# antgroup/ant-ray

Measured on NVIDIA H100. Metric: resnet50_ddp_train_images_per_sec, higher is better.
Workload: dtype bf16

## Files before the change

### ant-ray_b200/csrc/inst_norm.cu

```cuda
#include <algorithm>
#include <initializer_list>
#include <type_traits>

#include "norm_act.cuh"
#include "norm_infer.cuh"
#include "norm_kernels.cuh"
#include "norm_launch.h"
#include "norm_res.cuh"

namespace b200c {
namespace bn {

static int ceil_div(int a, int b) { return (a + b - 1) / b; }

static int last_pow2(unsigned n) {
  n |= (n >> 1);
  n |= (n >> 2);
  n |= (n >> 4);
  n |= (n >> 8);
  n |= (n >> 16);
  return std::max<int>(1, n - (n >> 1));
}

static void reduce_config(int reduction, int stride, dim3* block, dim3* grid) {
  int block_x = std::min(last_pow2(stride), kTileW);
  int block_y = std::min(last_pow2(ceil_div(reduction, kElemsPerThread)), kMaxBlock / block_x);
  if (block_x * block_y != kMaxBlock) block_x = std::min(last_pow2(stride), kMaxBlock / block_y);
  int grid_y = std::min(ceil_div(reduction, block_y * kElemsPerThread), kMaxHBlock);
  *block = dim3(block_x, block_y, 1);
  *grid = dim3(ceil_div(stride, block_x), grid_y < 8 ? 1 : grid_y, 1);
}

static_assert(kEwVec % kStatsVec == 0, "vec_ok covers the statistics kernel's vector width");
static bool vec_ok(int stride, const void* const* ptrs, int n) {
  if (stride % kEwVec) return false;
  for (int i = 0; i < n; i++)
    if (reinterpret_cast<uintptr_t>(ptrs[i]) % 16) return false;
  return true;
}

static void ew_config(int reduction, int stride, int vec, dim3* block, dim3* grid) {
  const int groups = stride / vec;
  const int bx = std::min(groups, kEwThreads);
  const int by = kEwThreads / bx;
  const int gx = ceil_div(groups, bx);
  const int gy = std::max(1, std::min(ceil_div(reduction, by), 4096 / gx));
  *block = dim3(bx, by, 1);
  *grid = dim3(gx, gy, 1);
}

constexpr int kSemaphores = kMaxChannels / kTileW;
constexpr size_t kSemaphoreBytes = (size_t)kSemaphores * 4;

// ... 18 lines not shown
template <int... Cs, typename F>
static auto with_const(int key, F&& f) {
  std::common_type_t<decltype(f(std::integral_constant<int, Cs>{}))...> kernel = nullptr;
  ((key == Cs ? void(kernel = f(std::integral_constant<int, Cs>{})) : void()), ...);
  return kernel;
}

using StatsKernel = void (*)(const bf16*, StatsOut, volatile float*, int*, int, int);
using SyncStatsKernel = void (*)(const bf16*, float*, float, volatile float*, int*, int, int);
using StatsDualKernel = void (*)(const bf16*, const bf16*, StatsOut, StatsOut, volatile float*, volatile float*, int*, int, int);
using TransformKernel = void (*)(const bf16*, const bf16*, bf16*, uint8_t*, const float*, const float*, const float*, const float*,
                                 const float*, const float*, const float*, const float*, int, int);
using PoolFwdKernel = void (*)(const bf16*, bf16*, uint8_t*, const float*, const float*, const float*, const float*, PoolDims, int, int);
using BwdReduceKernel = void (*)(const bf16*, const bf16*, const bf16*, const bf16*, const uint8_t*, bf16*, const float*, const float*,
                                 float*, float*, float*, float*, volatile float*, int*, PoolDims, const bf16*, const float*, const float*,
                                 float*, float*, float*, int, int);
using BwdElemtKernel = void (*)(const bf16*, const bf16*, const bf16*, const uint8_t*, const bf16*, bf16*, const float*, const float*,
                                const float*, const float*, const float*, const float*, float, const bf16*, bf16*, const float*,
                                const float*, const float*, const float*, int, int);

static StatsKernel stats_kernel(int vec) {
  return with_const<1, kStatsVec>(vec, [](auto v) -> StatsKernel { return k_bn_stats<decltype(v)::value>; });
}
static StatsDualKernel stats_dual_kernel(int vec) {
  return with_const<1, kStatsVec>(vec, [](auto v) -> StatsDualKernel { return k_bn_stats_dual<decltype(v)::value>; });
}
static SyncStatsKernel sync_stats_kernel(int vec) {
  return with_const<1, kStatsVec>(vec, [](auto v) -> SyncStatsKernel { return k_bn_sync_stats<decltype(v)::value>; });
}
static TransformKernel transform_kernel(int vec, int tail) {
  return with_const<1, kEwVec>(vec, [&](auto v) {
// ... 130 lines not shown
      load(res_infer_kernel<float>(vec, b));
      load(res_infer_kernel<bf16>(vec, b));
    }
  }
  return e;
}

constexpr cudaError_t kNoKernel = cudaErrorInvalidDeviceFunction;

static cudaError_t launch_stats(const FwdArgs& a, float* sync_row, cudaStream_t st) {
  Scratch s = carve(a.scratch, a.c);
  dim3 block, grid;
  reduce_config(a.m, a.c, &block, &grid);
  const int vec = vec_ok(a.c, &a.x, 1) ? kStatsVec : 1;
  block.x /= vec;
  const bf16* x = static_cast<const bf16*>(a.x);
  if (sync_row) {
    const SyncStatsKernel k = sync_stats_kernel(vec);
    if (!k) return kNoKernel;
    k<<<grid, block, 0, st>>>(x, sync_row, a.eps, s.staging, s.semaphores, a.m, a.c);
  } else {
    const StatsKernel k = stats_kernel(vec);
    if (!k) return kNoKernel;
    StatsOut o{a.save_mean, a.save_invstd, a.running_mean, a.running_var, a.num_batches_tracked, a.momentum,
               (float)((double)a.m / (double)(a.m - 1)), a.eps};
    k<<<grid, block, 0, st>>>(x, o, s.staging, s.semaphores, a.m, a.c);
  }
  return cudaGetLastError();
}

static cudaError_t launch_transform(const FwdArgs& a, cudaStream_t st) {
  const void* ptrs[3] = {a.x, a.y, a.identity ? a.identity : a.x};
  const int vec = vec_ok(a.c, ptrs, 3) ? kEwVec : 1;
  dim3 block, grid;
  ew_config(a.m, a.c, vec, &block, &grid);
  const TransformKernel k = transform_kernel(vec, !a.relu ? kTailNone : a.identity ? kTailAddRelu : kTailRelu);
  if (!k) return kNoKernel;
  k<<<grid, block, 0, st>>>(static_cast<const bf16*>(a.x), static_cast<const bf16*>(a.identity), static_cast<bf16*>(a.y),
                            static_cast<uint8_t*>(a.mask), a.save_mean, a.save_invstd, a.weight, a.bias, nullptr, nullptr, nullptr,
                            nullptr, a.m, a.c);
  return cudaGetLastError();
// ... 18 lines not shown
cudaError_t forward(const FwdArgs& a, cudaStream_t st) {
  const cudaError_t e = launch_stats(a, nullptr, st);
  if (e != cudaSuccess) return e;
  return a.pool_h ? launch_pool_fwd(a, st) : launch_transform(a, st);
}

static GradSrc grad_src(const BwdArgs& a, bool reduced) {
  if (!a.relu) return kGradDy;
  if (reduced && a.dy_masked) return kGradMasked;
  if (a.pool_h) return kGradPool;
  return a.mask ? kGradBits : kGradY;
}

static cudaError_t launch_bwd_reduce(const BwdArgs& a, cudaStream_t st) {
  Scratch s = carve(a.scratch, a.c);
  dim3 block, grid;
  reduce_config(a.m, a.c, &block, &grid);
  const GradSrc src = grad_src(a, false);
  const BwdReduceKernel k = bwd_reduce_kernel(src, false);
  if (!k) return kNoKernel;
  const void* mask = src == kGradPool ? a.argmax : a.mask;
  k<<<grid, block, 0, st>>>(static_cast<const bf16*>(a.x), static_cast<const bf16*>(a.dy), static_cast<const bf16*>(a.dy2),
                            static_cast<const bf16*>(a.y), static_cast<const uint8_t*>(mask), static_cast<bf16*>(a.dy_masked),
                            a.save_mean, a.save_invstd, s.sums, s.sums + a.c, a.grad_weight, a.grad_bias, s.staging, s.semaphores,
                            pool_dims(a.pool_h, a.pool_w), nullptr, nullptr, nullptr, nullptr, nullptr, nullptr, a.m, a.c);
  return cudaGetLastError();
}

static cudaError_t launch_bwd_elemt(const BwdArgs& a, cudaStream_t st) {
  Scratch s = carve(a.scratch, a.c);
  const GradSrc src = grad_src(a, true);
  const void* g = src == kGradMasked ? a.dy_masked : a.dy;
  const void* ptrs[5] = {a.x, a.dx, g, a.dy2 && src != kGradMasked ? a.dy2 : a.dy, a.y};
  const int vec = vec_ok(a.c, ptrs, src == kGradY ? 5 : 4) ? kEwVec : 1;
  dim3 block, grid;
  ew_config(a.m, a.c, vec, &block, &grid);
  const BwdElemtKernel k = bwd_elemt_kernel(vec, src, a.norm_fct != nullptr, false);
  if (!k) return kNoKernel;
  k<<<grid, block, 0, st>>>(static_cast<const bf16*>(g), static_cast<const bf16*>(a.dy2), static_cast<const bf16*>(a.y),
                            static_cast<const uint8_t*>(a.mask), static_cast<const bf16*>(a.x), static_cast<bf16*>(a.dx), a.save_mean,
// ... 8 lines not shown
}

static size_t dual_extra_offset(int c) { return (scratch_bytes(c) + 15) / 16 * 16; }
size_t dual_scratch_bytes(int c) { return dual_extra_offset(c) + (size_t)3 * c * kMaxHBlock * 4 + (size_t)c * 4; }
static float* dual_staging(void* scratch, int c) { return reinterpret_cast<float*>(static_cast<char*>(scratch) + dual_extra_offset(c)); }
static float* dual_sum_xmu2(void* scratch, int c) { return dual_staging(scratch, c) + (size_t)3 * c * kMaxHBlock; }

cudaError_t forward_dual(const FwdArgs& a, const FwdArgs& b, cudaStream_t st) {
  Scratch s = carve(a.scratch, a.c);
  dim3 block, grid;
  reduce_config(a.m, a.c, &block, &grid);
  const void* xs[2] = {a.x, b.x};
  const int svec = vec_ok(a.c, xs, 2) ? kStatsVec : 1;
  block.x /= svec;
  grid.z = 2;
  const StatsDualKernel ks = stats_dual_kernel(svec);
  if (!ks) return kNoKernel;
  StatsOut oa{a.save_mean, a.save_invstd, a.running_mean, a.running_var, a.num_batches_tracked, a.momentum,
              (float)((double)a.m / (double)(a.m - 1)), a.eps};
  StatsOut ob{b.save_mean, b.save_invstd, b.running_mean, b.running_var, b.num_batches_tracked, b.momentum,
              (float)((double)b.m / (double)(b.m - 1)), b.eps};
  ks<<<grid, block, 0, st>>>(static_cast<const bf16*>(a.x), static_cast<const bf16*>(b.x), oa, ob, s.staging,
                             dual_staging(a.scratch, a.c), s.semaphores, a.m, a.c);
  cudaError_t e = cudaGetLastError();
  if (e != cudaSuccess) return e;
  const void* ptrs[3] = {a.x, a.y, b.x};
  const int vec = vec_ok(a.c, ptrs, 3) ? kEwVec : 1;
  ew_config(a.m, a.c, vec, &block, &grid);
  const TransformKernel kt = transform_kernel(vec, kTailBnAddRelu);
  if (!kt) return kNoKernel;
  kt<<<grid, block, 0, st>>>(static_cast<const bf16*>(a.x), static_cast<const bf16*>(b.x), static_cast<bf16*>(a.y),
                             static_cast<uint8_t*>(a.mask), a.save_mean, a.save_invstd, a.weight, a.bias, b.save_mean, b.save_invstd,
                             b.weight, b.bias, a.m, a.c);
  return cudaGetLastError();
}

cudaError_t backward_dual(const BwdArgs& a, const BwdArgs& b, cudaStream_t st) {
  Scratch s = carve(a.scratch, a.c);
  float* sum2 = dual_sum_xmu2(a.scratch, a.c);
  const GradSrc src = a.mask ? kGradBits : kGradY;
  dim3 block, grid;
  reduce_config(a.m, a.c, &block, &grid);
  const BwdReduceKernel kr = bwd_reduce_kernel(src, true);
  if (!kr) return kNoKernel;
  kr<<<grid, block, 0, st>>>(static_cast<const bf16*>(a.x), static_cast<const bf16*>(a.dy), static_cast<const bf16*>(a.dy2),
                             static_cast<const bf16*>(a.y), static_cast<const uint8_t*>(a.mask), nullptr, a.save_mean, a.save_invstd,
                             s.sums, s.sums + a.c, a.grad_weight, a.grad_bias, s.staging, s.semaphores, pool_dims(0, 0),
                             static_cast<const bf16*>(b.x), b.save_mean, b.save_invstd, sum2, b.grad_weight, b.grad_bias, a.m, a.c);
  cudaError_t e = cudaGetLastError();
  if (e != cudaSuccess) return e;
  const void* ptrs[7] = {a.x, a.dx, a.dy, a.dy2 ? a.dy2 : a.dy, b.x, b.dx, a.y};
  const int vec = vec_ok(a.c, ptrs, src == kGradY ? 7 : 6) ? kEwVec : 1;
  ew_config(a.m, a.c, vec, &block, &grid);
  const BwdElemtKernel ke = bwd_elemt_kernel(vec, src, false, true);
  if (!ke) return kNoKernel;
  ke<<<grid, block, 0, st>>>(static_cast<const bf16*>(a.dy), static_cast<const bf16*>(a.dy2), static_cast<const bf16*>(a.y),
                             static_cast<const uint8_t*>(a.mask), static_cast<const bf16*>(a.x), static_cast<bf16*>(a.dx), a.save_mean,
                             a.save_invstd, a.weight, s.sums, s.sums + a.c, nullptr, (float)(1.0 / a.m), static_cast<const bf16*>(b.x),
                             static_cast<bf16*>(b.dx), b.save_mean, b.save_invstd, b.weight, sum2, a.m, a.c);
  return cudaGetLastError();
}

template <typename P>
static cudaError_t launch_infer(const InferArgs& a, cudaStream_t st) {
  auto p = [](const void* q) { return static_cast<const P*>(q); };
  const bf16* x = static_cast<const bf16*>(a.x);
  bf16* y = static_cast<bf16*>(a.y);
// ... 179 lines not shown
```

### ant-ray_b200/csrc/norm_kernels.cuh

```cuda
#pragma once
#include <cuda_bf16.h>
#include <cuda_runtime.h>
#include <stdint.h>

namespace b200c {
namespace bn {

constexpr int kMaxBlock = 512;
constexpr int kParallelLoads = 4;
constexpr int kElemsPerThread = 16;
constexpr int kTileW = 32;
constexpr int kMaxHBlock = 128;
constexpr int kStatsVec = 4;
constexpr int kEwThreads = 256;
constexpr int kEwVec = 8;

typedef __nv_bfloat16 bf16;

template <int V>
struct alignas(2 * V) BVec {
  bf16 v[V];
};


template <bool FUSE_NEW>
__device__ __forceinline__ void welford_merge_element(int& count, float& mean, float& m2n, const int& count_new,
                                                      const float& mean_new, const float& m2n_new) {
  float factor = float(1.0) / ::max(1, (count + count_new));
  float delta0 = mean - mean_new;
  const float c = count, c_new = count_new;
  mean = __fmul_rn(FUSE_NEW ? __fmaf_rn(mean_new, c_new, __fmul_rn(mean, c)) : __fmaf_rn(mean, c, __fmul_rn(mean_new, c_new)),
                   factor);
  m2n = __fadd_rn(m2n, __fmaf_rn(__fmul_rn(__fmul_rn(__fmul_rn(delta0, delta0), c_new), c), factor, m2n_new));
  count += count_new;
}

template <int V>
// ... 13 lines not shown
    }
    __syncthreads();
    if (threadIdx.y < offset && threadIdx.y + offset < blockDim.y) {
      auto address = address_base + offset * block_x;
#pragma unroll
      for (int k = 0; k < V; k++) {
        auto count_new = shmem_count[address + k];
        auto mean_new = shmem_mean[address + k];
        auto m2n_new = shmem_m2n[address + k];
        welford_merge_element<false>(count[k], mean[k], m2n[k], count_new, mean_new, m2n_new);
      }
    }
  }
}

__device__ __forceinline__ void merge_block_vertical_backward(float& sum_dy, float& sum_dy_xmu, float* shmem_sum_dy,
                                                              float* shmem_sum_dy_xmu) {
  auto address_base = threadIdx.x + threadIdx.y * blockDim.x;
#pragma unroll
  for (int offset = blockDim.y / 2; offset > 0; offset >>= 1) {
    if (threadIdx.y < offset * 2) {
      shmem_sum_dy[address_base] = sum_dy;
      shmem_sum_dy_xmu[address_base] = sum_dy_xmu;
    }
    __syncthreads();
    if (threadIdx.y < offset && threadIdx.y + offset < blockDim.y) {
      auto address = address_base + offset * blockDim.x;
      sum_dy += shmem_sum_dy[address];
      sum_dy_xmu += shmem_sum_dy_xmu[address];
    }
  }
}

struct StatsOut {
  float* save_mean;
  float* save_invstd;
  float* running_mean;
  float* running_var;
  long long* num_batches_tracked;
  float momentum, bessel, eps;
};

__device__ __forceinline__ void finish_stats(const StatsOut& o, int c, float mean_th, float m2_th, int count_th) {
  const float mean = mean_th;
  const float var = m2_th / count_th;
  const float momentum = o.momentum;
// ... 15 lines not shown
  for (int i = 0; i < PARALLEL_LOADS; i++) {
#pragma unroll
    for (int k = 0; k < V; k++) {
      x_mean[i][k] = 0.f;
      m_2_n[i][k] = 0.f;
    }
    count[i] = 0;
  }

  int inner_loop_stride = blockDim.y * gridDim.y;
  int m_offset = blockIdx.y * blockDim.y + threadIdx.y;
  int c_offset = (blockIdx.x * blockDim.x + threadIdx.x) * V;
  int loop_count = 1 + (reduction_size - 1) / (inner_loop_stride * PARALLEL_LOADS);
  const bool c_valid = c_offset < stride;

  for (int i = 0; i < loop_count; i++) {
    BVec<V> xv[PARALLEL_LOADS];
#pragma unroll
    for (int j = 0; j < PARALLEL_LOADS; j++) {
      const int m = m_offset + j * inner_loop_stride;
      if (c_valid && m < reduction_size) xv[j] = *reinterpret_cast<const BVec<V>*>(input + ((size_t)m * stride + c_offset));
    }
#pragma unroll
    for (int j = 0; j < PARALLEL_LOADS; j++) {
      float x_math[V];
      float x_count_inv;
      float is_valid;
      if (c_valid && m_offset < reduction_size) {
#pragma unroll
        for (int k = 0; k < V; k++) x_math[k] = __bfloat162float(xv[j].v[k]);
        count[j]++;
        x_count_inv = float(1) / count[j];
        is_valid = float(1);
      } else {
#pragma unroll
        for (int k = 0; k < V; k++) x_math[k] = float(0);
        x_count_inv = float(0);
        is_valid = float(0);
      }
      m_offset += inner_loop_stride;
#pragma unroll
      for (int k = 0; k < V; k++) {
        float delta0 = x_math[k] - x_mean[j][k];
        x_mean[j][k] = __fmaf_rn(delta0, x_count_inv, x_mean[j][k]);
        float delta1 = x_math[k] - x_mean[j][k];
        m_2_n[j][k] = __fmaf_rn(__fmul_rn(delta0, delta1), is_valid, m_2_n[j][k]);
      }
    }
  }
  float mean_th[V], m2_th[V];
  int count_th[V];
#pragma unroll
  for (int k = 0; k < V; k++) {
    count_th[k] = count[0];
    mean_th[k] = x_mean[0][k];
    m2_th[k] = m_2_n[0][k];
#pragma unroll
    for (int j = 1; j < PARALLEL_LOADS; j++) welford_merge_element<true>(count_th[k], mean_th[k], m2_th[k], count[j], x_mean[j][k], m_2_n[j][k]);
  }

  __shared__ float shmem_mean[kMaxBlock];
  __shared__ float shmem_m2n[kMaxBlock];
// ... 265 lines not shown
  if (a[0] == at) sum += __bfloat162float(v[0]);
  if (pw1 != pw0 && a[1] == at - 2) sum += __bfloat162float(v[1]);
  if (ph1 != ph0 && a[2] == at - 6) sum += __bfloat162float(v[2]);
  if (ph1 != ph0 && pw1 != pw0 && a[3] == at - 8) sum += __bfloat162float(v[3]);
  return __float2bfloat16(sum);
}

__device__ __forceinline__ bf16 relu_grad(bf16 dy, bf16 y) { return __bfloat162float(y) <= 0.f ? __float2bfloat16(0.f) : dy; }
__device__ __forceinline__ bf16 relu_grad_bit(bf16 dy, unsigned bit) { return bit ? dy : __float2bfloat16(0.f); }
__device__ __forceinline__ bf16 add_grads(bf16 a, bf16 b) { return __float2bfloat16(__bfloat162float(a) + __bfloat162float(b)); }

enum GradSrc { kGradMasked, kGradY, kGradBits, kGradDy, kGradPool };
constexpr int kGradSrcs = 5;

template <GradSrc G, bool DUAL>
__global__ void k_bn_bwd_reduce(const bf16* __restrict__ input, const bf16* __restrict__ grad_output,
                                const bf16* __restrict__ grad_output2, const bf16* __restrict__ output,
                                const uint8_t* __restrict__ mask, bf16* __restrict__ masked, const float* __restrict__ mean,
                                const float* __restrict__ inv_std, float* __restrict__ sum_dy_o, float* __restrict__ sum_dy_xmu_o,
                                float* __restrict__ grad_weight, float* __restrict__ grad_bias, volatile float* staging_data,
                                int* semaphores, const PoolDims pool, const bf16* __restrict__ input2,
                                const float* __restrict__ mean2, const float* __restrict__ inv_std2, float* __restrict__ sum_dy_xmu2_o,
                                float* __restrict__ grad_weight2, float* __restrict__ grad_bias2, const int reduction_size,
                                const int stride) {
  static_assert(G != kGradMasked, "the reduce kernel computes g");
  constexpr bool BITS = G == kGradBits;
  constexpr bool POOL = G == kGradPool;
  constexpr int PARALLEL_LOADS = kParallelLoads;
  float sum_dy[PARALLEL_LOADS];
  float sum_dy_xmu[PARALLEL_LOADS];
  float sum_dy_xmu2[PARALLEL_LOADS];
#pragma unroll
  for (int i = 0; i < PARALLEL_LOADS; i++) {
    sum_dy[i] = float(0);
    sum_dy_xmu[i] = float(0);
    sum_dy_xmu2[i] = float(0);
  }
  int inner_loop_stride = blockDim.y * gridDim.y;
  int m_offset = blockIdx.y * blockDim.y + threadIdx.y;
  int c_offset = blockIdx.x * blockDim.x + threadIdx.x;
  if (c_offset >= stride || m_offset >= reduction_size) return;

  int loop_count = 1 + (reduction_size - 1) / (inner_loop_stride * PARALLEL_LOADS);
  int address_base = m_offset * stride + c_offset;
  int address_increment = inner_loop_stride * stride;
  auto r_mean = mean[c_offset];
  auto factor = inv_std[c_offset];
  const float r_mean2 = DUAL ? mean2[c_offset] : 0.f;

  for (int i = 0; i < loop_count; i++) {
    bf16 dy_v[PARALLEL_LOADS], dy2_v[PARALLEL_LOADS], y_v[PARALLEL_LOADS], x_v[PARALLEL_LOADS], x2_v[PARALLEL_LOADS];
    uint8_t mask_v[PARALLEL_LOADS];
#pragma unroll
    for (int j = 0; j < PARALLEL_LOADS; j++) {
      if (m_offset + j * inner_loop_stride < reduction_size) {
        const int a = address_base + j * address_increment;
        if (POOL) dy_v[j] = pool_grad(grad_output, mask, pool, m_offset + j * inner_loop_stride, c_offset, stride);
        else dy_v[j] = grad_output[a];
        if (grad_output2) dy2_v[j] = grad_output2[a];
        if (BITS) mask_v[j] = mask[a >> 3];
        else if (G == kGradY) y_v[j] = output[a];
        x_v[j] = input[a];
        if (DUAL) x2_v[j] = input2[a];
      }
    }
    float x_input[PARALLEL_LOADS];
    float x_input2[PARALLEL_LOADS];
    float x_grad_output[PARALLEL_LOADS];
#pragma unroll
    for (int j = 0; j < PARALLEL_LOADS; j++) {
      if (c_offset < stride && m_offset < reduction_size) {
        const bf16 dy = !POOL && grad_output2 ? add_grads(dy_v[j], dy2_v[j]) : dy_v[j];
        const bf16 g = BITS ? relu_grad_bit(dy, (mask_v[j] >> (address_base & 7)) & 1u) : G == kGradY ? relu_grad(dy, y_v[j]) : dy;
        if (masked) masked[address_base] = g;
        x_input[j] = __bfloat162float(x_v[j]);
        x_input2[j] = DUAL ? __bfloat162float(x2_v[j]) : 0.f;
        x_grad_output[j] = __bfloat162float(g);
      } else {
        x_input[j] = float(0);
        x_input2[j] = float(0);
        x_grad_output[j] = float(0);
      }
      m_offset += inner_loop_stride;
      address_base += address_increment;
    }
#pragma unroll
    for (int j = 0; j < PARALLEL_LOADS; j++) {
      sum_dy[j] += x_grad_output[j];
      sum_dy_xmu[j] = __fmaf_rn(x_grad_output[j], x_input[j] - r_mean, sum_dy_xmu[j]);
      if (DUAL) sum_dy_xmu2[j] = __fmaf_rn(x_grad_output[j], x_input2[j] - r_mean2, sum_dy_xmu2[j]);
    }
  }
#pragma unroll
  for (int j = 1; j < PARALLEL_LOADS; j++) {
    sum_dy[0] += sum_dy[j];
    sum_dy_xmu[0] += sum_dy_xmu[j];
    if (DUAL) sum_dy_xmu2[0] += sum_dy_xmu2[j];
  }
  auto sum_dy_th = sum_dy[0];
  auto sum_dy_xmu_th = sum_dy_xmu[0];
  float sum_dy_xmu2_th = sum_dy_xmu2[0];

  __shared__ float shmem_sum_dy[kMaxBlock];
  __shared__ float shmem_sum_dy_xmu[kMaxBlock];
  auto merge = [&]() {
    merge_block_vertical_backward(sum_dy_th, sum_dy_xmu_th, shmem_sum_dy, shmem_sum_dy_xmu);
    if (DUAL) {
      __syncthreads();
      float unused = 0.f;
      merge_block_vertical_backward(sum_dy_xmu2_th, unused, shmem_sum_dy, shmem_sum_dy_xmu);
    }
  };
  merge();

  auto write_sums = [&]() {
    grad_bias[c_offset] = sum_dy_th;
    grad_weight[c_offset] = sum_dy_xmu_th * factor;
    sum_dy_o[c_offset] = sum_dy_th;
    sum_dy_xmu_o[c_offset] = sum_dy_xmu_th;
    if (DUAL) {
      grad_bias2[c_offset] = sum_dy_th;
      grad_weight2[c_offset] = sum_dy_xmu2_th * inv_std2[c_offset];
      sum_dy_xmu2_o[c_offset] = sum_dy_xmu2_th;
    }
  };
  if (gridDim.y > 1) {
    volatile float* staging_sum_dy = staging_data;
    volatile float* staging_sum_dy_xmu = &staging_data[stride * gridDim.y];
    volatile float* staging_sum_dy_xmu2 = &staging_data[2 * stride * gridDim.y];
    address_base = c_offset + blockIdx.y * stride;
    if (threadIdx.y == 0 && c_offset < stride) {
      staging_sum_dy[address_base] = sum_dy_th;
      staging_sum_dy_xmu[address_base] = sum_dy_xmu_th;
      if (DUAL) staging_sum_dy_xmu2[address_base] = sum_dy_xmu2_th;
    }
    __threadfence();
    __syncthreads();
    __shared__ bool is_last_block_done;
    if (threadIdx.x == 0 && threadIdx.y == 0) {
      int old = atomicAdd(&semaphores[blockIdx.x], 1);
      is_last_block_done = (old == (gridDim.y - 1));
      if (is_last_block_done) semaphores[blockIdx.x] = 0;
    }
    __syncthreads();
    if (is_last_block_done) {
      sum_dy_th = float(0.0);
      sum_dy_xmu_th = float(0.0);
      sum_dy_xmu2_th = float(0.0);
      for (int y = threadIdx.y; y < gridDim.y; y += blockDim.y) {
        address_base = c_offset + y * stride;
        sum_dy_th += (c_offset < stride ? staging_sum_dy[address_base] : float(0.0));
        sum_dy_xmu_th += (c_offset < stride ? staging_sum_dy_xmu[address_base] : float(0.0));
        if (DUAL) sum_dy_xmu2_th += (c_offset < stride ? staging_sum_dy_xmu2[address_base] : float(0.0));
      }
      merge();
      if (threadIdx.y == 0 && c_offset < stride) write_sums();
    }
  } else {
    if (blockIdx.y == 0 && threadIdx.y == 0 && c_offset < stride) write_sums();
  }
}

template <int V, GradSrc G, bool FCT_PTR, bool DUAL>
__global__ void __launch_bounds__(kEwThreads) k_bn_bwd_elemt(const bf16* __restrict__ grad_output, const bf16* __restrict__ grad_output2,
                                                             const bf16* __restrict__ output, const uint8_t* __restrict__ mask,
                                                             const bf16* __restrict__ input, bf16* __restrict__ grad_input,
                                                             const float* __restrict__ mean, const float* __restrict__ inv_std,
                                                             const float* __restrict__ weight, const float* __restrict__ sum_dy,
                                                             const float* __restrict__ sum_dy_xmu,
                                                             const float* __restrict__ norm_fct_ptr, const float norm_fct_value,
                                                             const bf16* __restrict__ input2, bf16* __restrict__ grad_input2,
                                                             const float* __restrict__ mean2, const float* __restrict__ inv_std2,
                                                             const float* __restrict__ weight2, const float* __restrict__ sum_dy_xmu2,
                                                             const int reduction_size, const int stride) {
  static_assert(!DUAL || (G == kGradY || G == kGradBits), "a dual tail derives g from dy and the ReLU");
// ... 48 lines not shown
```

Measured before the change: 5472.

## Pipeline BN stats and backward-reduce loads through cp.async shared-memory rings

The batch-norm statistics kernel and the backward reduce kernel now stage their global loads through a multi-stage shared-memory ring filled with cp.async, so loads for later iterations overlap with the Welford and gradient accumulation of the current one. The backward reduce kernel also gains a 4-wide channel vectorized path, selected at launch through a new vec argument, with dynamic shared memory sized by operand count. This aims to hide memory latency in these bandwidth-bound reductions. In exchange, each block uses more shared memory, which may lower occupancy, and the code adds more template paths.

Result: faster. 5648, median of 6 (+3.2%).

```diff
diff --git a/ant-ray_b200/csrc/inst_norm.cu b/ant-ray_b200/csrc/inst_norm.cu
--- a/ant-ray_b200/csrc/inst_norm.cu
+++ b/ant-ray_b200/csrc/inst_norm.cu
@@ -37,6 +37,38 @@
   for (int i = 0; i < n; i++)
     if (reinterpret_cast<uintptr_t>(ptrs[i]) % 16) return false;
   return true;
+}
+
+constexpr size_t kBlockSmem = 48 * 1024;
+constexpr size_t kStatsStaticSmem = 3 * kMaxBlock * 4 + 16;
+constexpr size_t kBwdStaticSmem = 2 * kMaxBlock * 4 + 16;
+
+static size_t stats_ring_bytes(dim3 block) {
+  return (size_t)kStatsStages * kParallelLoads * block.x * block.y * sizeof(BVec<kStatsVec>);
+}
+static_assert(kStatsStaticSmem + (size_t)kStatsStages * kParallelLoads * (kMaxBlock / kStatsVec) * sizeof(BVec<kStatsVec>) <= kBlockSmem,
+              "the statistics ring fits every block");
+
+static_assert(kBwdStaticSmem + (size_t)kBwdStagesWide * 5 * kParallelLoads * (kMaxBlock / kBwdVec) * sizeof(BVec<kBwdVec>) <= kBlockSmem &&
+                  kBwdStaticSmem + (size_t)kBwdStages * 2 * kParallelLoads * (kMaxBlock / kBwdVec) * sizeof(BVec<kBwdVec>) <= kBlockSmem,
+              "the backward ring fits every block: 2 stages of up to 5 operands, 3 of 2");
+struct BwdReduceLaunch {
+  dim3 block, grid;
+  int vec;
+  size_t smem;
+};
+static BwdReduceLaunch bwd_reduce_launch(int m, int c, GradSrc src, bool dy2, bool dual, const void* const* ptrs, int n) {
+  BwdReduceLaunch l;
+  reduce_config(m, c, &l.block, &l.grid);
+  l.vec = 1;
+  l.smem = 0;
+  if (src == kGradPool || !vec_ok(c, ptrs, n)) return l;
+  const int ops = bwd_ring_operands(src == kGradY, dy2, dual);
+  const size_t ring = (size_t)bwd_ring_stages(ops) * ops * kParallelLoads * (l.block.x / kBwdVec) * l.block.y * sizeof(BVec<kBwdVec>);
+  l.block.x /= kBwdVec;
+  l.vec = kBwdVec;
+  l.smem = ring;
+  return l;
 }
 
 static void ew_config(int reduction, int stride, int vec, dim3* block, dim3* grid) {
@@ -85,7 +117,7 @@
 using PoolFwdKernel = void (*)(const bf16*, bf16*, uint8_t*, const float*, const float*, const float*, const float*, PoolDims, int, int);
 using BwdReduceKernel = void (*)(const bf16*, const bf16*, const bf16*, const bf16*, const uint8_t*, bf16*, const float*, const float*,
                                  float*, float*, float*, float*, volatile float*, int*, PoolDims, const bf16*, const float*, const float*,
-                                 float*, float*, float*, int, int);
+                                 float*, float*, float*, int, int, int);
 using BwdElemtKernel = void (*)(const bf16*, const bf16*, const bf16*, const uint8_t*, const bf16*, bf16*, const float*, const float*,
                                 const float*, const float*, const float*, const float*, float, const bf16*, bf16*, const float*,
                                 const float*, const float*, const float*, int, int);
@@ -246,17 +278,18 @@
   reduce_config(a.m, a.c, &block, &grid);
   const int vec = vec_ok(a.c, &a.x, 1) ? kStatsVec : 1;
   block.x /= vec;
+  const size_t smem = vec == kStatsVec ? stats_ring_bytes(block) : 0;
   const bf16* x = static_cast<const bf16*>(a.x);
   if (sync_row) {
     const SyncStatsKernel k = sync_stats_kernel(vec);
     if (!k) return kNoKernel;
-    k<<<grid, block, 0, st>>>(x, sync_row, a.eps, s.staging, s.semaphores, a.m, a.c);
+    k<<<grid, block, smem, st>>>(x, sync_row, a.eps, s.staging, s.semaphores, a.m, a.c);
   } else {
     const StatsKernel k = stats_kernel(vec);
     if (!k) return kNoKernel;
     StatsOut o{a.save_mean, a.save_invstd, a.running_mean, a.running_var, a.num_batches_tracked, a.momentum,
                (float)((double)a.m / (double)(a.m - 1)), a.eps};
-    k<<<grid, block, 0, st>>>(x, o, s.staging, s.semaphores, a.m, a.c);
+    k<<<grid, block, smem, st>>>(x, o, s.staging, s.semaphores, a.m, a.c);
   }
   return cudaGetLastError();
 }
@@ -305,16 +338,16 @@
 
 static cudaError_t launch_bwd_reduce(const BwdArgs& a, cudaStream_t st) {
   Scratch s = carve(a.scratch, a.c);
-  dim3 block, grid;
-  reduce_config(a.m, a.c, &block, &grid);
   const GradSrc src = grad_src(a, false);
+  const void* ptrs[5] = {a.x, a.dy, a.dy2 ? a.dy2 : a.dy, src == kGradY ? a.y : a.dy, a.dy_masked ? a.dy_masked : a.dy};
+  const BwdReduceLaunch l = bwd_reduce_launch(a.m, a.c, src, a.dy2 != nullptr, false, ptrs, 5);
   const BwdReduceKernel k = bwd_reduce_kernel(src, false);
   if (!k) return kNoKernel;
   const void* mask = src == kGradPool ? a.argmax : a.mask;
-  k<<<grid, block, 0, st>>>(static_cast<const bf16*>(a.x), static_cast<const bf16*>(a.dy), static_cast<const bf16*>(a.dy2),
+  k<<<l.grid, l.block, l.smem, st>>>(static_cast<const bf16*>(a.x), static_cast<const bf16*>(a.dy), static_cast<const bf16*>(a.dy2),
                             static_cast<const bf16*>(a.y), static_cast<const uint8_t*>(mask), static_cast<bf16*>(a.dy_masked),
                             a.save_mean, a.save_invstd, s.sums, s.sums + a.c, a.grad_weight, a.grad_bias, s.staging, s.semaphores,
-                            pool_dims(a.pool_h, a.pool_w), nullptr, nullptr, nullptr, nullptr, nullptr, nullptr, a.m, a.c);
+                            pool_dims(a.pool_h, a.pool_w), nullptr, nullptr, nullptr, nullptr, nullptr, nullptr, a.m, a.c, l.vec);
   return cudaGetLastError();
 }
 
@@ -353,13 +386,14 @@
   const int svec = vec_ok(a.c, xs, 2) ? kStatsVec : 1;
   block.x /= svec;
   grid.z = 2;
+  const size_t smem = svec == kStatsVec ? stats_ring_bytes(block) : 0;
   const StatsDualKernel ks = stats_dual_kernel(svec);
   if (!ks) return kNoKernel;
   StatsOut oa{a.save_mean, a.save_invstd, a.running_mean, a.running_var, a.num_batches_tracked, a.momentum,
               (float)((double)a.m / (double)(a.m - 1)), a.eps};
   StatsOut ob{b.save_mean, b.save_invstd, b.running_mean, b.running_var, b.num_batches_tracked, b.momentum,
               (float)((double)b.m / (double)(b.m - 1)), b.eps};
-  ks<<<grid, block, 0, st>>>(static_cast<const bf16*>(a.x), static_cast<const bf16*>(b.x), oa, ob, s.staging,
+  ks<<<grid, block, smem, st>>>(static_cast<const bf16*>(a.x), static_cast<const bf16*>(b.x), oa, ob, s.staging,
                              dual_staging(a.scratch, a.c), s.semaphores, a.m, a.c);
   cudaError_t e = cudaGetLastError();
   if (e != cudaSuccess) return e;
@@ -378,18 +412,19 @@
   Scratch s = carve(a.scratch, a.c);
   float* sum2 = dual_sum_xmu2(a.scratch, a.c);
   const GradSrc src = a.mask ? kGradBits : kGradY;
-  dim3 block, grid;
-  reduce_config(a.m, a.c, &block, &grid);
+  const void* rptrs[5] = {a.x, a.dy, a.dy2 ? a.dy2 : a.dy, src == kGradY ? a.y : a.dy, b.x};
+  const BwdReduceLaunch l = bwd_reduce_launch(a.m, a.c, src, a.dy2 != nullptr, true, rptrs, 5);
   const BwdReduceKernel kr = bwd_reduce_kernel(src, true);
   if (!kr) return kNoKernel;
-  kr<<<grid, block, 0, st>>>(static_cast<const bf16*>(a.x), static_cast<const bf16*>(a.dy), static_cast<const bf16*>(a.dy2),
+  kr<<<l.grid, l.block, l.smem, st>>>(static_cast<const bf16*>(a.x), static_cast<const bf16*>(a.dy), static_cast<const bf16*>(a.dy2),
                              static_cast<const bf16*>(a.y), static_cast<const uint8_t*>(a.mask), nullptr, a.save_mean, a.save_invstd,
                              s.sums, s.sums + a.c, a.grad_weight, a.grad_bias, s.staging, s.semaphores, pool_dims(0, 0),
-                             static_cast<const bf16*>(b.x), b.save_mean, b.save_invstd, sum2, b.grad_weight, b.grad_bias, a.m, a.c);
+                             static_cast<const bf16*>(b.x), b.save_mean, b.save_invstd, sum2, b.grad_weight, b.grad_bias, a.m, a.c, l.vec);
   cudaError_t e = cudaGetLastError();
   if (e != cudaSuccess) return e;
   const void* ptrs[7] = {a.x, a.dx, a.dy, a.dy2 ? a.dy2 : a.dy, b.x, b.dx, a.y};
   const int vec = vec_ok(a.c, ptrs, src == kGradY ? 7 : 6) ? kEwVec : 1;
+  dim3 block, grid;
   ew_config(a.m, a.c, vec, &block, &grid);
   const BwdElemtKernel ke = bwd_elemt_kernel(vec, src, false, true);
   if (!ke) return kNoKernel;
diff --git a/ant-ray_b200/csrc/norm_kernels.cuh b/ant-ray_b200/csrc/norm_kernels.cuh
--- a/ant-ray_b200/csrc/norm_kernels.cuh
+++ b/ant-ray_b200/csrc/norm_kernels.cuh
@@ -2,6 +2,8 @@
 #include <cuda_bf16.h>
 #include <cuda_runtime.h>
 #include <stdint.h>
+
+#include <type_traits>
 
 namespace b200c {
 namespace bn {
@@ -12,6 +14,12 @@
 constexpr int kTileW = 32;
 constexpr int kMaxHBlock = 128;
 constexpr int kStatsVec = 4;
+constexpr int kBwdVec = 4;
+constexpr int kStatsStages = 4;
+constexpr unsigned kBwdStages = 3;
+constexpr unsigned kBwdStagesWide = 2;
+__host__ __device__ constexpr unsigned bwd_ring_stages(int ops) { return ops >= 3 ? kBwdStagesWide : kBwdStages; }
+__host__ __device__ constexpr int bwd_ring_operands(bool y, bool dy2, bool dual) { return 2 + dy2 + y + dual; }
 constexpr int kEwThreads = 256;
 constexpr int kEwVec = 8;
 
@@ -21,6 +29,19 @@
 struct alignas(2 * V) BVec {
   bf16 v[V];
 };
+
+__device__ __forceinline__ unsigned char* ring_smem() {
+  extern __shared__ __align__(16) unsigned char bn_ring[];
+  return bn_ring;
+}
+template <int BYTES>
+__device__ __forceinline__ void cp_async(void* smem, const void* gmem) {
+  asm volatile("cp.async.ca.shared.global [%0], [%1], %2;\n" ::"r"((unsigned)__cvta_generic_to_shared(smem)), "l"(gmem), "n"(BYTES)
+               : "memory");
+}
+__device__ __forceinline__ void cp_async_commit() { asm volatile("cp.async.commit_group;\n" ::: "memory"); }
+template <int N>
+__device__ __forceinline__ void cp_async_wait() { asm volatile("cp.async.wait_group %0;\n" ::"n"(N) : "memory"); }
 
 
 template <bool FUSE_NEW>
@@ -64,22 +85,38 @@
   }
 }
 
+template <int V>
+__device__ __forceinline__ void merge_block_vertical_backward(float (&sum_dy)[V], float (&sum_dy_xmu)[V], float* shmem_sum_dy,
+                                                              float* shmem_sum_dy_xmu) {
+  const int block_x = blockDim.x * V;
+  auto address_base = threadIdx.x * V + threadIdx.y * block_x;
+#pragma unroll
+  for (int offset = blockDim.y / 2; offset > 0; offset >>= 1) {
+    if (threadIdx.y < offset * 2) {
+#pragma unroll
+      for (int k = 0; k < V; k++) {
+        shmem_sum_dy[address_base + k] = sum_dy[k];
+        shmem_sum_dy_xmu[address_base + k] = sum_dy_xmu[k];
+      }
+    }
+    __syncthreads();
+    if (threadIdx.y < offset && threadIdx.y + offset < blockDim.y) {
+      auto address = address_base + offset * block_x;
+#pragma unroll
+      for (int k = 0; k < V; k++) {
+        sum_dy[k] += shmem_sum_dy[address + k];
+        sum_dy_xmu[k] += shmem_sum_dy_xmu[address + k];
+      }
+    }
+  }
+}
+
 __device__ __forceinline__ void merge_block_vertical_backward(float& sum_dy, float& sum_dy_xmu, float* shmem_sum_dy,
                                                               float* shmem_sum_dy_xmu) {
-  auto address_base = threadIdx.x + threadIdx.y * blockDim.x;
-#pragma unroll
-  for (int offset = blockDim.y / 2; offset > 0; offset >>= 1) {
-    if (threadIdx.y < offset * 2) {
-      shmem_sum_dy[address_base] = sum_dy;
-      shmem_sum_dy_xmu[address_base] = sum_dy_xmu;
-    }
-    __syncthreads();
-    if (threadIdx.y < offset && threadIdx.y + offset < blockDim.y) {
-      auto address = address_base + offset * blockDim.x;
-      sum_dy += shmem_sum_dy[address];
-      sum_dy_xmu += shmem_sum_dy_xmu[address];
-    }
-  }
+  float a[1] = {sum_dy}, b[1] = {sum_dy_xmu};
+  merge_block_vertical_backward<1>(a, b, shmem_sum_dy, shmem_sum_dy_xmu);
+  sum_dy = a[0];
+  sum_dy_xmu = b[0];
 }
 
 struct StatsOut {
@@ -125,38 +162,65 @@
   int loop_count = 1 + (reduction_size - 1) / (inner_loop_stride * PARALLEL_LOADS);
   const bool c_valid = c_offset < stride;
 
-  for (int i = 0; i < loop_count; i++) {
-    BVec<V> xv[PARALLEL_LOADS];
-#pragma unroll
-    for (int j = 0; j < PARALLEL_LOADS; j++) {
-      const int m = m_offset + j * inner_loop_stride;
-      if (c_valid && m < reduction_size) xv[j] = *reinterpret_cast<const BVec<V>*>(input + ((size_t)m * stride + c_offset));
-    }
-#pragma unroll
-    for (int j = 0; j < PARALLEL_LOADS; j++) {
-      float x_math[V];
-      float x_count_inv;
-      float is_valid;
-      if (c_valid && m_offset < reduction_size) {
-#pragma unroll
-        for (int k = 0; k < V; k++) x_math[k] = __bfloat162float(xv[j].v[k]);
-        count[j]++;
-        x_count_inv = float(1) / count[j];
-        is_valid = float(1);
-      } else {
-#pragma unroll
-        for (int k = 0; k < V; k++) x_math[k] = float(0);
-        x_count_inv = float(0);
-        is_valid = float(0);
-      }
-      m_offset += inner_loop_stride;
-#pragma unroll
-      for (int k = 0; k < V; k++) {
-        float delta0 = x_math[k] - x_mean[j][k];
-        x_mean[j][k] = __fmaf_rn(delta0, x_count_inv, x_mean[j][k]);
-        float delta1 = x_math[k] - x_mean[j][k];
-        m_2_n[j][k] = __fmaf_rn(__fmul_rn(delta0, delta1), is_valid, m_2_n[j][k]);
-      }
+  auto update = [&](int j, const BVec<V>* xv) {
+    float x_math[V];
+    float x_count_inv;
+    float is_valid;
+    if (c_valid && m_offset < reduction_size) {
+      const BVec<V> x = *xv;
+#pragma unroll
+      for (int k = 0; k < V; k++) x_math[k] = __bfloat162float(x.v[k]);
+      count[j]++;
+      x_count_inv = float(1) / count[j];
+      is_valid = float(1);
+    } else {
+#pragma unroll
+      for (int k = 0; k < V; k++) x_math[k] = float(0);
+      x_count_inv = float(0);
+      is_valid = float(0);
+    }
+    m_offset += inner_loop_stride;
+#pragma unroll
+    for (int k = 0; k < V; k++) {
+      float delta0 = x_math[k] - x_mean[j][k];
+      x_mean[j][k] = __fmaf_rn(delta0, x_count_inv, x_mean[j][k]);
+      float delta1 = x_math[k] - x_mean[j][k];
+      m_2_n[j][k] = __fmaf_rn(__fmul_rn(delta0, delta1), is_valid, m_2_n[j][k]);
+    }
+  };
+
+  if constexpr (V == 1) {
+    for (int i = 0; i < loop_count; i++) {
+      BVec<V> xv[PARALLEL_LOADS];
+#pragma unroll
+      for (int j = 0; j < PARALLEL_LOADS; j++) {
+        const int m = m_offset + j * inner_loop_stride;
+        if (c_valid && m < reduction_size) xv[j] = *reinterpret_cast<const BVec<V>*>(input + ((size_t)m * stride + c_offset));
+      }
+#pragma unroll
+      for (int j = 0; j < PARALLEL_LOADS; j++) update(j, &xv[j]);
+    }
+  } else {
+    constexpr unsigned D = kStatsStages;
+    const int threads = blockDim.x * blockDim.y;
+    BVec<V>* ring = reinterpret_cast<BVec<V>*>(ring_smem()) + threadIdx.y * blockDim.x + threadIdx.x;
+    const int first_row = m_offset;
+    auto issue = [&](unsigned it) {
+      BVec<V>* slot = ring + (it % D) * PARALLEL_LOADS * threads;
+      int m = first_row + (int)it * PARALLEL_LOADS * inner_loop_stride;
+#pragma unroll
+      for (int j = 0; j < PARALLEL_LOADS; j++, m += inner_loop_stride)
+        if (c_valid && m < reduction_size) cp_async<sizeof(BVec<V>)>(slot + j * threads, input + ((size_t)m * stride + c_offset));
+      cp_async_commit();
+    };
+#pragma unroll
+    for (unsigned it = 0; it < D - 1; it++) issue(it);
+    for (unsigned i = 0; i < (unsigned)loop_count; i++) {
+      issue(i + D - 1);
+      cp_async_wait<D - 1>();
+      const BVec<V>* slot = ring + (i % D) * PARALLEL_LOADS * threads;
+#pragma unroll
+      for (int j = 0; j < PARALLEL_LOADS; j++) update(j, slot + j * threads);
     }
   }
   float mean_th[V], m2_th[V];
@@ -452,7 +516,7 @@
 constexpr int kGradSrcs = 5;
 
 template <GradSrc G, bool DUAL>
-__global__ void k_bn_bwd_reduce(const bf16* __restrict__ input, const bf16* __restrict__ grad_output,
+__global__ void __launch_bounds__(kMaxBlock) k_bn_bwd_reduce(const bf16* __restrict__ input, const bf16* __restrict__ grad_output,
                                 const bf16* __restrict__ grad_output2, const bf16* __restrict__ output,
                                 const uint8_t* __restrict__ mask, bf16* __restrict__ masked, const float* __restrict__ mean,
                                 const float* __restrict__ inv_std, float* __restrict__ sum_dy_o, float* __restrict__ sum_dy_xmu_o,
@@ -460,143 +524,238 @@
                                 int* semaphores, const PoolDims pool, const bf16* __restrict__ input2,
                                 const float* __restrict__ mean2, const float* __restrict__ inv_std2, float* __restrict__ sum_dy_xmu2_o,
                                 float* __restrict__ grad_weight2, float* __restrict__ grad_bias2, const int reduction_size,
-                                const int stride) {
+                                const int stride, const int vec) {
   static_assert(G != kGradMasked, "the reduce kernel computes g");
   constexpr bool BITS = G == kGradBits;
   constexpr bool POOL = G == kGradPool;
   constexpr int PARALLEL_LOADS = kParallelLoads;
-  float sum_dy[PARALLEL_LOADS];
-  float sum_dy_xmu[PARALLEL_LOADS];
-  float sum_dy_xmu2[PARALLEL_LOADS];
-#pragma unroll
-  for (int i = 0; i < PARALLEL_LOADS; i++) {
-    sum_dy[i] = float(0);
-    sum_dy_xmu[i] = float(0);
-    sum_dy_xmu2[i] = float(0);
-  }
-  int inner_loop_stride = blockDim.y * gridDim.y;
-  int m_offset = blockIdx.y * blockDim.y + threadIdx.y;
-  int c_offset = blockIdx.x * blockDim.x + threadIdx.x;
-  if (c_offset >= stride || m_offset >= reduction_size) return;
-
-  int loop_count = 1 + (reduction_size - 1) / (inner_loop_stride * PARALLEL_LOADS);
-  int address_base = m_offset * stride + c_offset;
-  int address_increment = inner_loop_stride * stride;
-  auto r_mean = mean[c_offset];
-  auto factor = inv_std[c_offset];
-  const float r_mean2 = DUAL ? mean2[c_offset] : 0.f;
-
-  for (int i = 0; i < loop_count; i++) {
-    bf16 dy_v[PARALLEL_LOADS], dy2_v[PARALLEL_LOADS], y_v[PARALLEL_LOADS], x_v[PARALLEL_LOADS], x2_v[PARALLEL_LOADS];
-    uint8_t mask_v[PARALLEL_LOADS];
-#pragma unroll
-    for (int j = 0; j < PARALLEL_LOADS; j++) {
-      if (m_offset + j * inner_loop_stride < reduction_size) {
-        const int a = address_base + j * address_increment;
-        if (POOL) dy_v[j] = pool_grad(grad_output, mask, pool, m_offset + j * inner_loop_stride, c_offset, stride);
-        else dy_v[j] = grad_output[a];
-        if (grad_output2) dy2_v[j] = grad_output2[a];
-        if (BITS) mask_v[j] = mask[a >> 3];
-        else if (G == kGradY) y_v[j] = output[a];
-        x_v[j] = input[a];
-        if (DUAL) x2_v[j] = input2[a];
-      }
-    }
-    float x_input[PARALLEL_LOADS];
-    float x_input2[PARALLEL_LOADS];
-    float x_grad_output[PARALLEL_LOADS];
-#pragma unroll
-    for (int j = 0; j < PARALLEL_LOADS; j++) {
-      if (c_offset < stride && m_offset < reduction_size) {
-        const bf16 dy = !POOL && grad_output2 ? add_grads(dy_v[j], dy2_v[j]) : dy_v[j];
-        const bf16 g = BITS ? relu_grad_bit(dy, (mask_v[j] >> (address_base & 7)) & 1u) : G == kGradY ? relu_grad(dy, y_v[j]) : dy;
-        if (masked) masked[address_base] = g;
-        x_input[j] = __bfloat162float(x_v[j]);
-        x_input2[j] = DUAL ? __bfloat162float(x2_v[j]) : 0.f;
-        x_grad_output[j] = __bfloat162float(g);
+  __shared__ float shmem_sum_dy[kMaxBlock];
+  __shared__ float shmem_sum_dy_xmu[kMaxBlock];
+  __shared__ bool is_last_block_done;
+
+  auto body = [&](auto vec_c) {
+    constexpr int V = decltype(vec_c)::value;
+    float sum_dy[PARALLEL_LOADS][V];
+    float sum_dy_xmu[PARALLEL_LOADS][V];
+    float sum_dy_xmu2[PARALLEL_LOADS][V];
+#pragma unroll
+    for (int i = 0; i < PARALLEL_LOADS; i++) {
+#pragma unroll
+      for (int k = 0; k < V; k++) {
+        sum_dy[i][k] = float(0);
+        sum_dy_xmu[i][k] = float(0);
+        sum_dy_xmu2[i][k] = float(0);
+      }
+    }
+    int inner_loop_stride = blockDim.y * gridDim.y;
+    int m_offset = blockIdx.y * blockDim.y + threadIdx.y;
+    int c_offset = (blockIdx.x * blockDim.x + threadIdx.x) * V;
+    if (c_offset >= stride || m_offset >= reduction_size) return;
+
+    int loop_count = 1 + (reduction_size - 1) / (inner_loop_stride * PARALLEL_LOADS);
+    int address_base = m_offset * stride + c_offset;
+    int address_increment = inner_loop_stride * stride;
+    float r_mean[V], factor[V], r_mean2[V];
+#pragma unroll
+    for (int k = 0; k < V; k++) {
+      r_mean[k] = mean[c_offset + k];
+      factor[k] = inv_std[c_offset + k];
+      r_mean2[k] = DUAL ? mean2[c_offset + k] : 0.f;
+    }
+
+    auto consume = [&](int j, const BVec<V>* dy_p, const BVec<V>* dy2_p, const BVec<V>* y_p, uint8_t mask_byte, const BVec<V>* x_p,
+                       const BVec<V>* x2_p) {
+      float x_input[V], x_input2[V], x_grad_output[V];
+      if (m_offset < reduction_size) {
+        const unsigned bits = BITS ? mask_byte >> (address_base & 7) : 0u;
+        BVec<V> gv;
+#pragma unroll
+        for (int k = 0; k < V; k++) {
+          const bf16 dy = !POOL && grad_output2 ? add_grads(dy_p->v[k], dy2_p->v[k]) : dy_p->v[k];
+          gv.v[k] = BITS ? relu_grad_bit(dy, (bits >> k) & 1u) : G == kGradY ? relu_grad(dy, y_p->v[k]) : dy;
+          x_input[k] = __bfloat162float(x_p->v[k]);
+          x_input2[k] = DUAL ? __bfloat162float(x2_p->v[k]) : 0.f;
+          x_grad_output[k] = __bfloat162float(gv.v[k]);
+        }
+        if (masked) *reinterpret_cast<BVec<V>*>(masked + address_base) = gv;
       } else {
-        x_input[j] = float(0);
-        x_input2[j] = float(0);
-        x_grad_output[j] = float(0);
+#pragma unroll
+        for (int k = 0; k < V; k++) {
+          x_input[k] = float(0);
+          x_input2[k] = float(0);
+          x_grad_output[k] = float(0);
+        }
       }
       m_offset += inner_loop_stride;
       address_base += address_increment;
-    }
-#pragma unroll
-    for (int j = 0; j < PARALLEL_LOADS; j++) {
-      sum_dy[j] += x_grad_output[j];
-      sum_dy_xmu[j] = __fmaf_rn(x_grad_output[j], x_input[j] - r_mean, sum_dy_xmu[j]);
-      if (DUAL) sum_dy_xmu2[j] = __fmaf_rn(x_grad_output[j], x_input2[j] - r_mean2, sum_dy_xmu2[j]);
-    }
-  }
-#pragma unroll
-  for (int j = 1; j < PARALLEL_LOADS; j++) {
-    sum_dy[0] += sum_dy[j];
-    sum_dy_xmu[0] += sum_dy_xmu[j];
-    if (DUAL) sum_dy_xmu2[0] += sum_dy_xmu2[j];
-  }
-  auto sum_dy_th = sum_dy[0];
-  auto sum_dy_xmu_th = sum_dy_xmu[0];
-  float sum_dy_xmu2_th = sum_dy_xmu2[0];
-
-  __shared__ float shmem_sum_dy[kMaxBlock];
-  __shared__ float shmem_sum_dy_xmu[kMaxBlock];
-  auto merge = [&]() {
-    merge_block_vertical_backward(sum_dy_th, sum_dy_xmu_th, shmem_sum_dy, shmem_sum_dy_xmu);
-    if (DUAL) {
+#pragma unroll
+      for (int k = 0; k < V; k++) {
+        sum_dy[j][k] += x_grad_output[k];
+        sum_dy_xmu[j][k] = __fmaf_rn(x_grad_output[k], x_input[k] - r_mean[k], sum_dy_xmu[j][k]);
+        if (DUAL) sum_dy_xmu2[j][k] = __fmaf_rn(x_grad_output[k], x_input2[k] - r_mean2[k], sum_dy_xmu2[j][k]);
+      }
+    };
+
+    if constexpr (V == 1) {
+      for (int i = 0; i < loop_count; i++) {
+        BVec<V> dy_v[PARALLEL_LOADS], dy2_v[PARALLEL_LOADS], y_v[PARALLEL_LOADS], x_v[PARALLEL_LOADS], x2_v[PARALLEL_LOADS];
+        uint8_t mask_v[PARALLEL_LOADS];
+#pragma unroll
+        for (int j = 0; j < PARALLEL_LOADS; j++) {
+          if (m_offset + j * inner_loop_stride < reduction_size) {
+            const int a = address_base + j * address_increment;
+            if (POOL) dy_v[j].v[0] = pool_grad(grad_output, mask, pool, m_offset + j * inner_loop_stride, c_offset, stride);
+            else dy_v[j].v[0] = grad_output[a];
+            if (grad_output2) dy2_v[j].v[0] = grad_output2[a];
+            if (BITS) mask_v[j] = mask[a >> 3];
+            else if (G == kGradY) y_v[j].v[0] = output[a];
+            x_v[j].v[0] = input[a];
+            if (DUAL) x2_v[j].v[0] = input2[a];
+          }
+        }
+#pragma unroll
+        for (int j = 0; j < PARALLEL_LOADS; j++) consume(j, &dy_v[j], &dy2_v[j], &y_v[j], mask_v[j], &x_v[j], &x2_v[j]);
+      }
+    } else {
+      const int ops = bwd_ring_operands(G == kGradY, grad_output2 != nullptr, DUAL);
+      auto ring_walk = [&](auto stages_c) {
+        constexpr unsigned D = decltype(stages_c)::value;
+        const int threads = blockDim.x * blockDim.y;
+        const int op_dy2 = 2, op_y = op_dy2 + (grad_output2 != nullptr), op_x2 = op_y + (G == kGradY);
+        BVec<V>* ring = reinterpret_cast<BVec<V>*>(ring_smem()) + threadIdx.y * blockDim.x + threadIdx.x;
+        auto stage = [&](unsigned it) { return ring + (it % D) * ops * PARALLEL_LOADS * threads; };
+        const int first_row = m_offset;
+        const int iteration_rows = PARALLEL_LOADS * inner_loop_stride;
+        auto issue = [&](unsigned it) {
+          BVec<V>* slot = stage(it);
+          int m = first_row + (int)it * iteration_rows;
+#pragma unroll
+          for (int j = 0; j < PARALLEL_LOADS; j++, m += inner_loop_stride, slot += threads) {
+            if (m < reduction_size) {
+              const size_t a = (size_t)m * stride + c_offset;
+              cp_async<sizeof(BVec<V>)>(slot, grad_output + a);
+              cp_async<sizeof(BVec<V>)>(slot + PARALLEL_LOADS * threads, input + a);
+              if (grad_output2) cp_async<sizeof(BVec<V>)>(slot + op_dy2 * PARALLEL_LOADS * threads, grad_output2 + a);
+              if (G == kGradY) cp_async<sizeof(BVec<V>)>(slot + op_y * PARALLEL_LOADS * threads, output + a);
+              if (DUAL) cp_async<sizeof(BVec<V>)>(slot + op_x2 * PARALLEL_LOADS * threads, input2 + a);
+            }
+          }
+          cp_async_commit();
+        };
+        uint8_t mask_next[PARALLEL_LOADS];
+        auto load_mask = [&](unsigned it) {
+          int m = first_row + (int)it * iteration_rows;
+#pragma unroll
+          for (int j = 0; j < PARALLEL_LOADS; j++, m += inner_loop_stride)
+            if (m < reduction_size) mask_next[j] = mask[((size_t)m * stride + c_offset) >> 3];
+        };
+        if (BITS) load_mask(0);
+#pragma unroll
+        for (unsigned it = 0; it < D - 1; it++) issue(it);
+        for (unsigned i = 0; i < (unsigned)loop_count; i++) {
+          issue(i + D - 1);
+          uint8_t mask_v[PARALLEL_LOADS];
+#pragma unroll
+          for (int j = 0; j < PARALLEL_LOADS; j++) mask_v[j] = mask_next[j];
+          if (BITS) load_mask(i + 1);
+          cp_async_wait<D - 1>();
+          const BVec<V>* slot = stage(i);
+#pragma unroll
+          for (int j = 0; j < PARALLEL_LOADS; j++, slot += threads)
+            consume(j, slot, slot + op_dy2 * PARALLEL_LOADS * threads, slot + op_y * PARALLEL_LOADS * threads, mask_v[j],
+                    slot + PARALLEL_LOADS * threads, slot + op_x2 * PARALLEL_LOADS * threads);
+        }
+      };
+      if (DUAL || bwd_ring_stages(ops) == kBwdStagesWide) ring_walk(std::integral_constant<unsigned, kBwdStagesWide>{});
+      else ring_walk(std::integral_constant<unsigned, kBwdStages>{});
+    }
+
+    float sum_dy_th[V], sum_dy_xmu_th[V], sum_dy_xmu2_th[V];
+#pragma unroll
+    for (int k = 0; k < V; k++) {
+#pragma unroll
+      for (int j = 1; j < PARALLEL_LOADS; j++) {
+        sum_dy[0][k] += sum_dy[j][k];
+        sum_dy_xmu[0][k] += sum_dy_xmu[j][k];
+        if (DUAL) sum_dy_xmu2[0][k] += sum_dy_xmu2[j][k];
+      }
+      sum_dy_th[k] = sum_dy[0][k];
+      sum_dy_xmu_th[k] = sum_dy_xmu[0][k];
+      sum_dy_xmu2_th[k] = sum_dy_xmu2[0][k];
+    }
+
+    auto merge = [&]() {
+      merge_block_vertical_backward<V>(sum_dy_th, sum_dy_xmu_th, shmem_sum_dy, shmem_sum_dy_xmu);
+      if (DUAL) {
+        __syncthreads();
+        float unused[V] = {};
+        merge_block_vertical_backward<V>(sum_dy_xmu2_th, unused, shmem_sum_dy, shmem_sum_dy_xmu);
+      }
+    };
+    merge();
+
+    auto write_sums = [&]() {
+#pragma unroll
+      for (int k = 0; k < V; k++) {
+        const int c = c_offset + k;
+        grad_bias[c] = sum_dy_th[k];
+        grad_weight[c] = sum_dy_xmu_th[k] * factor[k];
+        sum_dy_o[c] = sum_dy_th[k];
+        sum_dy_xmu_o[c] = sum_dy_xmu_th[k];
+        if (DUAL) {
+          grad_bias2[c] = sum_dy_th[k];
+          grad_weight2[c] = sum_dy_xmu2_th[k] * inv_std2[c];
+          sum_dy_xmu2_o[c] = sum_dy_xmu2_th[k];
+        }
+      }
+    };
+    if (gridDim.y > 1) {
+      volatile float* staging_sum_dy = staging_data;
+      volatile float* staging_sum_dy_xmu = &staging_data[stride * gridDim.y];
+      volatile float* staging_sum_dy_xmu2 = &staging_data[2 * stride * gridDim.y];
+      address_base = c_offset + blockIdx.y * stride;
+      if (threadIdx.y == 0 && c_offset < stride) {
+#pragma unroll
+        for (int k = 0; k < V; k++) {
+          staging_sum_dy[address_base + k] = sum_dy_th[k];
+          staging_sum_dy_xmu[address_base + k] = sum_dy_xmu_th[k];
+          if (DUAL) staging_sum_dy_xmu2[address_base + k] = sum_dy_xmu2_th[k];
+        }
+      }
+      __threadfence();
       __syncthreads();
-      float unused = 0.f;
-      merge_block_vertical_backward(sum_dy_xmu2_th, unused, shmem_sum_dy, shmem_sum_dy_xmu);
+      if (threadIdx.x == 0 && threadIdx.y == 0) {
+        int old = atomicAdd(&semaphores[blockIdx.x], 1);
+        is_last_block_done = (old == (gridDim.y - 1));
+        if (is_last_block_done) semaphores[blockIdx.x] = 0;
+      }
+      __syncthreads();
+      if (is_last_block_done) {
+#pragma unroll
+        for (int k = 0; k < V; k++) {
+          sum_dy_th[k] = float(0.0);
+          sum_dy_xmu_th[k] = float(0.0);
+          sum_dy_xmu2_th[k] = float(0.0);
+        }
+        for (int y = threadIdx.y; y < gridDim.y; y += blockDim.y) {
+          address_base = c_offset + y * stride;
+#pragma unroll
+          for (int k = 0; k < V; k++) {
+            sum_dy_th[k] += (c_offset < stride ? staging_sum_dy[address_base + k] : float(0.0));
+            sum_dy_xmu_th[k] += (c_offset < stride ? staging_sum_dy_xmu[address_base + k] : float(0.0));
+            if (DUAL) sum_dy_xmu2_th[k] += (c_offset < stride ? staging_sum_dy_xmu2[address_base + k] : float(0.0));
+          }
+        }
+        merge();
+        if (threadIdx.y == 0 && c_offset < stride) write_sums();
+      }
+    } else {
+      if (blockIdx.y == 0 && threadIdx.y == 0 && c_offset < stride) write_sums();
     }
   };
-  merge();
-
-  auto write_sums = [&]() {
-    grad_bias[c_offset] = sum_dy_th;
-    grad_weight[c_offset] = sum_dy_xmu_th * factor;
-    sum_dy_o[c_offset] = sum_dy_th;
-    sum_dy_xmu_o[c_offset] = sum_dy_xmu_th;
-    if (DUAL) {
-      grad_bias2[c_offset] = sum_dy_th;
-      grad_weight2[c_offset] = sum_dy_xmu2_th * inv_std2[c_offset];
-      sum_dy_xmu2_o[c_offset] = sum_dy_xmu2_th;
-    }
-  };
-  if (gridDim.y > 1) {
-    volatile float* staging_sum_dy = staging_data;
-    volatile float* staging_sum_dy_xmu = &staging_data[stride * gridDim.y];
-    volatile float* staging_sum_dy_xmu2 = &staging_data[2 * stride * gridDim.y];
-    address_base = c_offset + blockIdx.y * stride;
-    if (threadIdx.y == 0 && c_offset < stride) {
-      staging_sum_dy[address_base] = sum_dy_th;
-      staging_sum_dy_xmu[address_base] = sum_dy_xmu_th;
-      if (DUAL) staging_sum_dy_xmu2[address_base] = sum_dy_xmu2_th;
-    }
-    __threadfence();
-    __syncthreads();
-    __shared__ bool is_last_block_done;
-    if (threadIdx.x == 0 && threadIdx.y == 0) {
-      int old = atomicAdd(&semaphores[blockIdx.x], 1);
-      is_last_block_done = (old == (gridDim.y - 1));
-      if (is_last_block_done) semaphores[blockIdx.x] = 0;
-    }
-    __syncthreads();
-    if (is_last_block_done) {
-      sum_dy_th = float(0.0);
-      sum_dy_xmu_th = float(0.0);
-      sum_dy_xmu2_th = float(0.0);
-      for (int y = threadIdx.y; y < gridDim.y; y += blockDim.y) {
-        address_base = c_offset + y * stride;
-        sum_dy_th += (c_offset < stride ? staging_sum_dy[address_base] : float(0.0));
-        sum_dy_xmu_th += (c_offset < stride ? staging_sum_dy_xmu[address_base] : float(0.0));
-        if (DUAL) sum_dy_xmu2_th += (c_offset < stride ? staging_sum_dy_xmu2[address_base] : float(0.0));
-      }
-      merge();
-      if (threadIdx.y == 0 && c_offset < stride) write_sums();
-    }
-  } else {
-    if (blockIdx.y == 0 && threadIdx.y == 0 && c_offset < stride) write_sums();
-  }
+  if constexpr (POOL) body(std::integral_constant<int, 1>{});
+  else if (vec == kBwdVec) body(std::integral_constant<int, kBwdVec>{});
+  else body(std::integral_constant<int, 1>{});
 }
 
 template <int V, GradSrc G, bool FCT_PTR, bool DUAL>
```
